# JeffWang987/MVSTER

Measured on AMD Instinct MI355X. Metric: depth-maps/sec (DTU 512×640, 5-view, 4-stage) at 1/2/4/8 MI355X, higher is better.
Workload: dtype f32; 1 GPU; DTU mid 512x640, 5 views, 4-stage cascade 8/8/4/4 hyp, B=1 eval, 1 depth map(s) per step per GPU; launch=hipGraph replay, parallelism=replicas x1, depth_maps_in_flight_per_gpu=2

## Files before the change

mvster_amd/csrc/conv_args.hpp:

```cpp
#pragma once
#include "common.hpp"

namespace mvconv {

typedef float f32x4v __attribute__((ext_vector_type(4)));

constexpr int kMaxTaps = 128;
constexpr int kMaxClasses = 8;

struct ConvArgs {
    const float* in;
    const float* wpk;
    const float* scale;
    const float* shift;
    const float* skip;
    const float* zeros;
    const float* prob_w;
    const float* prob_b;
    float* out;
    int B, Di, Hi, Wi;
    int Do, Ho, Wo;
    int DoF, HoF, WoF;
    int sd, sh, sw;
    int cin;
    int cout;
    int ntile_total;
    int relu;
    int skip_mode;
    int nclass;
    int kd[kMaxClasses], kh[kMaxClasses], kw[kMaxClasses];
    int pd[kMaxClasses], ph[kMaxClasses], pw[kMaxClasses];
    int od[kMaxClasses], oh[kMaxClasses], ow[kMaxClasses];
    int osd, osh, osw;
    int nsteps[kMaxClasses];
    int all_inside[kMaxClasses];
    long woff[kMaxClasses];
    unsigned div_mul[3], div_shr[3];
    unsigned in_bytes;
};

__device__ __forceinline__ unsigned fast_div(unsigned n, unsigned d, unsigned mul, unsigned shr) {
    return d == 1 ? n : (__umulhi(n, mul) >> shr);
}

static inline void find_divisor(unsigned d, unsigned& mul, unsigned& shr) {
    if (d <= 1) { mul = 0; shr = 0; return; }
    int lg = 31 - __builtin_clz(d);
    if (d & (d - 1)) ++lg;
    const int p = 31 + lg;
    mul = (unsigned)(((1ull << p) + d - 1) / d);
    shr = (unsigned)(p - 32);
}

typedef __attribute__((address_space(3))) void lds_void;
typedef unsigned u32x4v __attribute__((ext_vector_type(4)));

struct PersArgs {
    unsigned tiles_x, tiles_y, ntiles;
    unsigned out_bytes;
    int prio;
    unsigned mul[3], shr[3], one[3];
};

struct TilePos { int b, zo, ty0, tx0; };

template <int MT, int KW, int SW, int KD>
struct PersGeom {
    static constexpr int TY = 2 * MT;
    static constexpr int KH = KW;
    static constexpr int PW = 31 * SW + KW;
    static constexpr int PH = (TY - 1) * SW + KH;
    static constexpr int ROWS = KD * PH;
    static constexpr int PWH = (PW + 1) / 2;
    static constexpr int ROWSLOTS = SW == 1 ? PW * 2 : PWH * 4;
    static constexpr int USED = ROWS * ROWSLOTS;
    static constexpr int NBLK = (USED + 63) / 64;
    static constexpr int PLANE = ((NBLK * 64 + 7) & ~7) + 4;
};

static inline bool fill_pers_args(const ConvArgs& a, int TY, PersArgs& p) {
    p.tiles_x = (unsigned)((a.Wo + 31) / 32);
    p.tiles_y = (unsigned)((a.Ho + TY - 1) / TY);
    const long ntiles = (long)p.tiles_x * p.tiles_y * a.Do * a.B;
    const long out_bytes = (long)a.B * a.DoF * a.HoF * a.WoF * a.cout * 4;
    if (ntiles >= (1L << 30) || a.in_bytes >= (1u << 31) || out_bytes >= (1L << 31)) return false;
    p.ntiles = (unsigned)ntiles;
    p.out_bytes = (unsigned)out_bytes;
    p.prio = 0;
    const unsigned divisors[3] = {p.tiles_x, p.tiles_y, (unsigned)a.Do};
    for (int i = 0; i < 3; ++i) {
        find_divisor(divisors[i], p.mul[i], p.shr[i]);
        p.one[i] = divisors[i] == 1 ? ~0u : 0u;
    }
    return true;
}

int num_cus();

static inline bool allow_big_lds(const void* kern, unsigned long& done) {
    int dev = 0;
    if (hipGetDevice(&dev) != hipSuccess) return false;
    if (dev >= 0 && dev < 64 && ((done >> dev) & 1ul)) return true;
    if (hipFuncSetAttribute(kern, hipFuncAttributeMaxDynamicSharedMemorySize, 160 * 1024) != hipSuccess) return false;
    if (dev >= 0 && dev < 64) done |= 1ul << dev;
    return true;
}

int dispatch_pers(const ConvArgs& a, int mt, int nt, int wpc, hipStream_t s);
int dispatch_pp(const ConvArgs& a, int mt, int nt, hipStream_t s);
int dispatch_wino(const ConvArgs& a, int nt, int wpc, bool ring, hipStream_t s);
int dispatch_b3(const ConvArgs& a, int mt, int wpc, hipStream_t s);
int dispatch_1x1(const ConvArgs& a, int mt, int wpc, hipStream_t s);

int dispatch_deconv_select_mfma(const float* in, const float* w, const float* scale, const float* shift, const float* skip,
                                const float* prob_w, const float* prob_b, const float* hypo, float* attn, float* depth,
                                float* conf, float* inv_min, float* inv_max, float* logits_out, int B, int D, int Hi, int Wi,
                                int relu, float split_itv, hipStream_t s);

}
```

mvster_amd/csrc/conv_mfma.hip:

```cpp
#include <stdlib.h>

#include "conv_args.hpp"

namespace {

using namespace mvconv;

typedef unsigned u32x4v __attribute__((ext_vector_type(4)));

#ifdef MVSTER_TIMELINE
__device__ unsigned long long* g_tl = nullptr;
#define MV_TL(k)                                                                                              \
    do {                                                                                                      \
        __builtin_amdgcn_sched_barrier(0);                                                                    \
        if (g_tl && (threadIdx.x & 63) == 0)                                                                  \
            g_tl[((size_t)blockIdx.x * 4 + (threadIdx.x >> 6)) * 8 + (k)] = __builtin_amdgcn_s_memtime();     \
        __builtin_amdgcn_sched_barrier(0);                                                                    \
    } while (0)
#define MV_TL_ID()                                                                                            \
    do {                                                                                                      \
        if (g_tl && (threadIdx.x & 63) == 0) {                                                                \
            g_tl[((size_t)blockIdx.x * 4 + (threadIdx.x >> 6)) * 8 + 6] = __builtin_amdgcn_s_getreg(63492);   \
            g_tl[((size_t)blockIdx.x * 4 + (threadIdx.x >> 6)) * 8 + 7] = __builtin_amdgcn_s_getreg(63508);   \
        }                                                                                                     \
    } while (0)
#else
#define MV_TL(k)
#define MV_TL_ID()
#endif

__device__ __forceinline__ void epilogue_store(const ConvArgs& a, f32x4v v, int n0, long opix, int b, int oy, int ox,
                                               const f32x4v sc, const f32x4v sh) {
    const bool vec = (n0 + 3 < a.cout) && ((a.cout & 3) == 0);
#pragma unroll
    for (int j = 0; j < 4; ++j) {
        v[j] = fmaf(v[j], sc[j], sh[j]);
        if (a.relu) v[j] = fmaxf(v[j], 0.0f);
    }
    if (a.prob_w) {
        if (a.skip_mode == 1) {
            const f32x4v k = *reinterpret_cast<const f32x4v*>(a.skip + opix * a.cout + n0);
#pragma unroll
            for (int j = 0; j < 4; ++j) v[j] += k[j];
        }
        float part = v[0] * a.prob_w[n0];
#pragma unroll
        for (int j = 1; j < 4; ++j) part = fmaf(v[j], a.prob_w[n0 + j], part);
        const float other = __shfl_xor(part, 16);
        if (n0 == 0) a.out[opix] = (part + other) + a.prob_b[0];
        return;
    }
    float* op = a.out + opix * a.cout + n0;
    if (vec) {
        if (a.skip_mode == 1) {
            const f32x4v k = *reinterpret_cast<const f32x4v*>(a.skip + opix * a.cout + n0);
#pragma unroll
            for (int j = 0; j < 4; ++j) v[j] += k[j];
        } else if (a.skip_mode == 2) {
            const int hh = a.HoF / 2, wh = a.WoF / 2;
            const mv::Lerp ly = mv::make_lerp(oy, hh, a.HoF), lx = mv::make_lerp(ox, wh, a.WoF);
            const float* sk = a.skip + (long)b * hh * wh * a.cout + n0;
            const f32x4v k00 = *reinterpret_cast<const f32x4v*>(sk + ((long)ly.i0 * wh + lx.i0) * a.cout);
            const f32x4v k01 = *reinterpret_cast<const f32x4v*>(sk + ((long)ly.i0 * wh + lx.i1) * a.cout);
            const f32x4v k10 = *reinterpret_cast<const f32x4v*>(sk + ((long)ly.i1 * wh + lx.i0) * a.cout);
            const f32x4v k11 = *reinterpret_cast<const f32x4v*>(sk + ((long)ly.i1 * wh + lx.i1) * a.cout);
#pragma unroll
            for (int j = 0; j < 4; ++j) v[j] = mv::bilerp(ly, lx, k00[j], k01[j], k10[j], k11[j]) + v[j];
        }
        *reinterpret_cast<f32x4v*>(op) = v;
    } else {
        for (int j = 0; j < 4; ++j) {
            if (n0 + j >= a.cout) break;
            float r = v[j];
            if (a.skip_mode == 1) r += a.skip[opix * a.cout + n0 + j];
            op[j] = r;
        }
    }
}

__device__ __forceinline__ void epilogue_store(const ConvArgs& a, f32x4v v, int n0, long opix, int b, int oy, int ox) {
    epilogue_store(a, v, n0, opix, b, oy, ox, *reinterpret_cast<const f32x4v*>(a.scale + n0),
                   *reinterpret_cast<const f32x4v*>(a.shift + n0));
}

constexpr int conv_min_waves(int mt, int nt) {
    const int t = mt * nt;
    return t <= 2 ? 5 : (t <= 4 ? 4 : (t <= 8 ? 3 : 2));
}

template <int CIN, int MT, int NT, bool SPLITK>
__global__ void __launch_bounds__(256, conv_min_waves(MT, NT)) conv_mfma_kernel(ConvArgs a) {
    static_assert(CIN % 4 == 0 && (CIN >= 16 ? CIN % 16 == 0 : 16 % CIN == 0), "channel packing");
    __shared__ f32x4v red[SPLITK ? 3 * MT * NT * 64 : 1];
    __shared__ int lut_ofs[kMaxTaps];
    __shared__ int lut_zyx[kMaxTaps];

    const int cls = blockIdx.z;
    const int KD = a.kd[cls], KH = a.kh[cls], KW = a.kw[cls];
    const int ntaps = KD * KH * KW;
    for (int t = threadIdx.x; t < ntaps; t += blockDim.x) {
        const int kx = t % KW, ky = (t / KW) % KH, kz = t / (KW * KH);
        lut_ofs[t] = (kz * a.Hi + ky) * a.Wi + kx;
        lut_zyx[t] = kz | (ky << 8) | (kx << 16);
    }
    __syncthreads();

    const int lane = threadIdx.x & 63;
    const int wave = threadIdx.x >> 6;
    const int lm = lane & 15;
    const int lq = lane >> 4;
    const unsigned Mtot = (unsigned)(a.B * a.Do * a.Ho * a.Wo);
    const int nt0 = blockIdx.y * NT;
    const unsigned ntiles = (Mtot + 15u) >> 4;
    const unsigned ngroups = SPLITK ? (ntiles + MT - 1) / MT : (ntiles + 4 * MT - 1) / (4 * MT);
    for (unsigned grp0 = blockIdx.x; grp0 < ngroups; grp0 += gridDim.x) {
    const unsigned grp = gridDim.x == ngroups ? xcd_remap(grp0, ngroups) : grp0;
    const unsigned tile0 = SPLITK ? grp * MT : (grp * 4u + wave) * MT;
    if (!SPLITK && tile0 * 16u >= Mtot) break;

    int iz0[MT], iy0[MT], ix0[MT];
    int pin0[MT];
    int opix[MT];
    int oyx[MT];
#pragma unroll
    for (int mt = 0; mt < MT; ++mt) {
        unsigned m = (tile0 + mt) * 16u + lm;
        const bool ok = m < Mtot;
        if (!ok) m = 0;
        unsigned r = fast_div(m, a.Wo, a.div_mul[0], a.div_shr[0]);
        const int x = (int)(m - r * (unsigned)a.Wo);
        unsigned r2 = fast_div(r, a.Ho, a.div_mul[1], a.div_shr[1]);
        const int y = (int)(r - r2 * (unsigned)a.Ho);
        const unsigned b = fast_div(r2, a.Do, a.div_mul[2], a.div_shr[2]);
        const int z = (int)(r2 - b * (unsigned)a.Do);
        iz0[mt] = ok ? z * a.sd - a.pd[cls] : -(1 << 20);
        iy0[mt] = y * a.sh - a.ph[cls];
        ix0[mt] = x * a.sw - a.pw[cls];
        pin0[mt] = (((int)b * a.Di + (ok ? iz0[mt] : 0)) * a.Hi + iy0[mt]) * a.Wi + ix0[mt];
        const int oz = z * a.osd + a.od[cls], oy = y * a.osh + a.oh[cls], ox = x * a.osw + a.ow[cls];
        opix[mt] = ok ? (((int)b * a.DoF + oz) * a.HoF + oy) * a.WoF + ox : -1;
        oyx[mt] = (oy << 16) | ox;
    }

    f32x4v acc[MT][NT];
#pragma unroll
    for (int mt = 0; mt < MT; ++mt)
#pragma unroll
        for (int nt = 0; nt < NT; ++nt) acc[mt][nt] = (f32x4v){0.f, 0.f, 0.f, 0.f};

    const float* wp = a.wpk + a.woff[cls] + ((long)nt0 * 64 + lane) * 4;
    const long wstep = (long)a.ntile_total * 256;
    const int nsteps_all = a.nsteps[cls];
    const int kfirst = SPLITK ? wave : 0, kstride = SPLITK ? 4 : 1;
    const int nsteps = SPLITK ? (nsteps_all - wave + 3) / 4 : nsteps_all;

    const __amdgpu_buffer_rsrc_t in_rsrc =
        __builtin_amdgcn_make_buffer_rsrc(const_cast<float*>(a.in), (short)0, (int)a.in_bytes, 0x00020000);
    const bool no_pad = a.all_inside[cls] != 0;
    f32x4v af[MT], bf[NT];
    auto load_step = [&](int si, f32x4v (&A)[MT], f32x4v (&Bv)[NT]) {
        const int s = kfirst + si * kstride;
        const int kk = s * 16 + lq * 4;
        const int tap = kk / CIN;
        const int c = kk % CIN;
        const bool tap_ok = tap < ntaps;
        const int tt = tap_ok ? tap : 0;
        const int ofs = lut_ofs[tt];
        const int zyx = lut_zyx[tt];
        const int kz = zyx & 255, ky = (zyx >> 8) & 255, kx = zyx >> 16;
#pragma unroll
        for (int mt = 0; mt < MT; ++mt) {
            bool ok = tap_ok && iz0[mt] > -(1 << 19);
            if (!no_pad)
                ok = ok && (unsigned)(iz0[mt] + kz) < (unsigned)a.Di && (unsigned)(iy0[mt] + ky) < (unsigned)a.Hi &&
                     (unsigned)(ix0[mt] + kx) < (unsigned)a.Wi;
            const unsigned off = ok ? (unsigned)((pin0[mt] + ofs) * CIN + c) * 4u : 0xFFFFFFF0u;
            A[mt] = __builtin_bit_cast(f32x4v, __builtin_amdgcn_raw_buffer_load_b128(in_rsrc, off, 0, 0));
        }
#pragma unroll
        for (int nt = 0; nt < NT; ++nt)
            Bv[nt] = *reinterpret_cast<const f32x4v*>(wp + (long)s * wstep + (long)nt * 256);
    };

    auto mma_step = [&](const f32x4v (&A)[MT], const f32x4v (&Bv)[NT]) {
#pragma unroll
        for (int j = 0; j < 4; ++j)
#pragma unroll
            for (int mt = 0; mt < MT; ++mt)
#pragma unroll
                for (int nt = 0; nt < NT; ++nt)
                    acc[mt][nt] = __builtin_amdgcn_mfma_f32_16x16x4f32(Bv[nt][j], A[mt][j], acc[mt][nt], 0, 0, 0);
    };

    f32x4v ag[MT], bg[NT];
    if (nsteps > 0) {
        load_step(0, af, bf);
        int s = 0;
        for (; s + 2 <= nsteps; s += 2) {
            load_step(s + 1, ag, bg);
            mma_step(af, bf);
            load_step(s + 2 < nsteps ? s + 2 : nsteps - 1, af, bf);
            mma_step(ag, bg);
        }
        if (s < nsteps) mma_step(af, bf);
    }

    if (SPLITK) {
        if (wave > 0) {
#pragma unroll
            for (int mt = 0; mt < MT; ++mt)
#pragma unroll
                for (int nt = 0; nt < NT; ++nt) red[((wave - 1) * MT * NT + mt * NT + nt) * 64 + lane] = acc[mt][nt];
        }
        __syncthreads();
        if (wave > 0) return;
#pragma unroll
        for (int w = 0; w < 3; ++w)
#pragma unroll
            for (int mt = 0; mt < MT; ++mt)
#pragma unroll
                for (int nt = 0; nt < NT; ++nt) {
                    const f32x4v r = red[(w * MT * NT + mt * NT + nt) * 64 + lane];
#pragma unroll
                    for (int j = 0; j < 4; ++j) acc[mt][nt][j] += r[j];
                }
    }

#pragma unroll
    for (int mt = 0; mt < MT; ++mt) {
        if (opix[mt] < 0) continue;
        const int b = a.skip_mode == 2 ? opix[mt] / (a.DoF * a.HoF * a.WoF) : 0;
#pragma unroll
        for (int nt = 0; nt < NT; ++nt) {
            const int n0 = (nt0 + nt) * 16 + lq * 4;
            if (n0 >= a.cout) continue;
            epilogue_store(a, acc[mt][nt], n0, opix[mt], b, oyx[mt] >> 16, oyx[mt] & 0xffff);
        }
    }
    }
}

template <int CIN, int MT, int NT, bool SPLITK>
int launch(const ConvArgs& a, hipStream_t s) {
    const long Mtot = (long)a.B * a.Do * a.Ho * a.Wo;
    if (Mtot >= (1L << 31) || (long)a.B * a.Di * a.Hi * a.Wi >= (1L << 31)) return MVSTER_ERR_SHAPE;
    const long tiles = (Mtot + 15) / 16;
    const long per_block = SPLITK ? MT : 4 * MT;
    long gx = (tiles + per_block - 1) / per_block;
    dim3 grid((unsigned)gx, a.ntile_total / NT, a.nclass);
    MV_NOTE_KERNEL("conv_mfma_kernel<%d, %d, %d, %s>", CIN, MT, NT, SPLITK ? "true" : "false");
    hipLaunchKernelGGL((conv_mfma_kernel<CIN, MT, NT, SPLITK>), grid, dim3(256), 0, s, a);
    return mv_check_launch();
}

template <int CIN>
int dispatch_tiles(const ConvArgs& a, int MT, int NT, bool splitk, hipStream_t s) {
    if (splitk) {
        if constexpr (CIN >= 16) {
#define MV_S(M_, N_) if (MT == M_ && NT == N_) return launch<CIN, M_, N_, true>(a, s);
            MV_S(1, 1) MV_S(1, 2) MV_S(1, 4) MV_S(2, 1) MV_S(2, 2)
#undef MV_S
        }
        return MVSTER_ERR_UNSUPPORTED;
    }
#define MV_T(M_, N_) if (MT == M_ && NT == N_) return launch<CIN, M_, N_, false>(a, s);
    MV_T(1, 1) MV_T(2, 1) MV_T(4, 1) MV_T(1, 2) MV_T(2, 2) MV_T(4, 2) MV_T(1, 4) MV_T(2, 4) MV_T(4, 4)
    if constexpr (CIN == 64) {
        MV_T(1, 5) MV_T(2, 5) MV_T(4, 5)
        MV_T(1, 3) MV_T(2, 3) MV_T(4, 3) MV_T(1, 9) MV_T(2, 9)
    }
#undef MV_T
    return MVSTER_ERR_UNSUPPORTED;
}

struct LdsDivs {
    unsigned mul[6], shr[6];
};
constexpr int kMaxStage = 12;
__device__ __forceinline__ int patch_plane(int npix) { return ((npix * 2 + 7) & ~7) + 4; }
static const bool g_no_wlds = MV_PROBE_ENV("MVSTER_NO_WLDS") != nullptr;

template <int MT, int NT, int KW, int NG, int WN>
__global__ void __launch_bounds__(256) conv_lds_kernel(ConvArgs a, int tiles_x, int tiles_y, LdsDivs dv) {
    extern __shared__ __attribute__((aligned(16))) float patch_raw[];
    MV_TL(0);
    MV_TL_ID();
    f32x4v* patch_base = reinterpret_cast<f32x4v*>(patch_raw);
    f32x4v* wl = patch_base + NG * 1024 + 32;
    constexpr int TY = 2 * MT;
    const int KD = a.kd[0], KH = a.kh[0];
    const int PW = 31 * a.sw + KW, PH = (TY - 1) * a.sh + KH;
    const int CIN = a.cin, nchunks = CIN >> 4;
    const int plane = patch_plane(KD * PH * PW);

    unsigned bid = xcd_remap(blockIdx.x, gridDim.x);
    unsigned q = fast_div(bid, tiles_x, dv.mul[0], dv.shr[0]);
    const int tile_x = bid - q * tiles_x; bid = q;
    q = fast_div(bid, tiles_y, dv.mul[1], dv.shr[1]);
    const int tile_y = bid - q * tiles_y; bid = q;
    q = fast_div(bid, a.Do, dv.mul[2], dv.shr[2]);
    const int zo = bid - q * a.Do;
    const int b = q;
    const int ty0 = tile_y * TY, tx0 = tile_x * 32;
    const int nt0 = blockIdx.y * NT;

    const int lane = threadIdx.x & 63, wave = threadIdx.x >> 6;
    const int lm = lane & 15, lq = lane >> 4;

    const bool split = a.sw == 2;
    const int PWH = (PW + 1) >> 1;
    const int npix = KD * PH * PW;
    int goff[NG], gslot[NG];
#pragma unroll
    for (int g = 0; g < NG; ++g) {
        const unsigned pix = threadIdx.x + g * 256;
        int off = -1;
        gslot[g] = (int)pix;
        if ((int)pix < npix) {
            const unsigned prow = fast_div(pix, PW, dv.mul[3], dv.shr[3]);
            const int px = pix - prow * PW;
            if (split) gslot[g] = (int)(prow * PW) + (px & 1) * PWH + (px >> 1);
            const int pz = fast_div(prow, PH, dv.mul[4], dv.shr[4]);
            const int py = prow - pz * PH;
            const int iz = zo * a.sd - a.pd[0] + pz, iy = ty0 * a.sh - a.ph[0] + py, ix = tx0 * a.sw - a.pw[0] + px;
            if ((unsigned)iz < (unsigned)a.Di && (unsigned)iy < (unsigned)a.Hi && (unsigned)ix < (unsigned)a.Wi)
                off = (((b * a.Di + iz) * a.Hi + iy) * a.Wi + ix) * CIN;
        }
        goff[g] = off;
    }
    const long zero_off = a.zeros - a.in;

    const float* wp = a.wpk + ((long)nt0 * 64 + lane) * 4;
    const long wstep = (long)a.ntile_total * 256;

    f32x4v stg[NG * 4];
    constexpr bool WL = WN > 0;
    f32x4v wst[WL ? WN : 1];
    const int nW = KD * KH * KW * NT * 64;
    auto stage_load = [&](int ch) {
#pragma unroll
        for (int i = 0; i < NG * 4; ++i) {
            const int o = goff[i >> 2];
            const long off = o >= 0 ? (long)o + ch * 16 + (i & 3) * 4 : zero_off;
            stg[i] = *reinterpret_cast<const f32x4v*>(a.in + off);
        }
        if (WL) {
#pragma unroll
            for (int i = 0; i < WN; ++i) {
                const int idx = min((int)threadIdx.x + i * 256, nW - 1);
                const int t = idx / (NT * 64), rem = idx - t * (NT * 64);
                wst[i] = *reinterpret_cast<const f32x4v*>(a.wpk + (long)(t * nchunks + ch) * wstep + ((long)nt0 * 64 + rem) * 4);
            }
        }
    };
    auto stage_store = [&](f32x4v* dst) {
#pragma unroll
        for (int i = 0; i < NG * 4; ++i) {
            const int pix = threadIdx.x + (i >> 2) * 256, quad = i & 3;
            if (pix < npix) dst[(quad >> 1) * plane + gslot[i >> 2] * 2 + (quad & 1)] = stg[i];
        }
        if (WL) {
#pragma unroll
            for (int i = 0; i < WN; ++i) wl[threadIdx.x + i * 256] = wst[i];
        }
    };
    stage_load(0);
    int abase[MT];
#pragma unroll
    for (int mt = 0; mt < MT; ++mt) {
        const int t = wave * MT + mt;
        const int row = t >> 1, xs = t & 1;
        abase[mt] = ((row * a.sh) * PW + (xs * 16 + lm) * (split ? 1 : a.sw)) * 2 + (lq >> 1) * plane + (lq & 1);
    }
    int kxo[KW];
#pragma unroll
    for (int kx = 0; kx < KW; ++kx) kxo[kx] = split ? ((kx & 1) * PWH + (kx >> 1)) * 2 : kx * 2;

    f32x4v acc[MT][NT];
#pragma unroll
    for (int mt = 0; mt < MT; ++mt)
#pragma unroll
        for (int nt = 0; nt < NT; ++nt) acc[mt][nt] = (f32x4v){0.f, 0.f, 0.f, 0.f};

    f32x4v scv[NT], shv[NT];
#pragma unroll
    for (int nt = 0; nt < NT; ++nt) {
        const int n0 = min((nt0 + nt) * 16 + lq * 4, a.ntile_total * 16 - 4);
        scv[nt] = *reinterpret_cast<const f32x4v*>(a.scale + n0);
        shv[nt] = *reinterpret_cast<const f32x4v*>(a.shift + n0);
    }
    MV_TL(1);
    stage_store(patch_base);
    MV_TL(2);
    __syncthreads();
    MV_TL(3);
    for (int ch = 0; ch < nchunks; ++ch) {
        const f32x4v* patch = patch_base;
        if (ch + 1 < nchunks) stage_load(ch + 1);
        const int kz_lo = max(0, a.pd[0] - zo * a.sd), kz_hi = min(KD, a.Di + a.pd[0] - zo * a.sd);
        const int r_first = kz_lo * KH, nrows = kz_hi * KH;
        auto load_row = [&](int r, f32x4v (&A)[KW][MT], f32x4v (&Bv)[KW][NT]) {
            const int kz = fast_div(r, KH, dv.mul[5], dv.shr[5]), ky = r - kz * KH;
            const int rowoff = (kz * PH + ky) * PW * 2;
            const float* w = wp + (long)(r * KW * nchunks + ch) * wstep;
#pragma unroll
            for (int kx = 0; kx < KW; ++kx) {
#pragma unroll
                for (int mt = 0; mt < MT; ++mt) A[kx][mt] = patch[abase[mt] + rowoff + kxo[kx]];
#pragma unroll
                for (int nt = 0; nt < NT; ++nt)
                    Bv[kx][nt] = WL ? wl[((r * KW + kx) * NT + nt) * 64 + lane]
                                    : *reinterpret_cast<const f32x4v*>(w + (long)kx * nchunks * wstep + nt * 256);
            }
        };
        auto mma_row = [&](const f32x4v (&A)[KW][MT], const f32x4v (&Bv)[KW][NT]) {
#pragma unroll
            for (int kx = 0; kx < KW; ++kx)
#pragma unroll
                for (int j = 0; j < 4; ++j)
#pragma unroll
                    for (int mt = 0; mt < MT; ++mt)
#pragma unroll
                        for (int nt = 0; nt < NT; ++nt)
                            acc[mt][nt] = __builtin_amdgcn_mfma_f32_16x16x4f32(Bv[kx][nt][j], A[kx][mt][j], acc[mt][nt], 0, 0, 0);
        };
        f32x4v a0[KW][MT], b0[KW][NT], a1[KW][MT], b1[KW][NT];
        load_row(r_first, a0, b0);
        int r = r_first;
        for (; r + 2 <= nrows; r += 2) {
            load_row(r + 1, a1, b1);
            mma_row(a0, b0);
            load_row(r + 2 < nrows ? r + 2 : nrows - 1, a0, b0);
            mma_row(a1, b1);
        }
        if (r < nrows) mma_row(a0, b0);
        if (ch + 1 < nchunks) {
            __syncthreads();
            stage_store(patch_base);
            __syncthreads();
        }
    }

    MV_TL(4);
#pragma unroll
    for (int mt = 0; mt < MT; ++mt) {
        const int t = wave * MT + mt;
        const int y = ty0 + (t >> 1), x = tx0 + (t & 1) * 16 + lm;
        if (y >= a.Ho || x >= a.Wo) continue;
        const long opix = (((long)b * a.Do + zo) * a.Ho + y) * a.Wo + x;
#pragma unroll
        for (int nt = 0; nt < NT; ++nt) {
            const int n0 = (nt0 + nt) * 16 + lq * 4;
            if (n0 >= a.cout) continue;
            epilogue_store(a, acc[mt][nt], n0, opix, b, y, x, scv[nt], shv[nt]);
        }
    }
    MV_TL(5);
}

template <int MT, int NT, int KW, int NG>
int launch_lds_ng(const ConvArgs& a, int tiles_x, int tiles_y, hipStream_t s) {
    const long blocks = (long)tiles_x * tiles_y * a.Do * a.B;
    if (blocks >= (1L << 31) || (long)a.B * a.Di * a.Hi * a.Wi * a.cin >= (1L << 31)) return MVSTER_ERR_SHAPE;
    dim3 grid((unsigned)blocks, a.ntile_total / NT, 1);
    LdsDivs dv;
    const unsigned divisors[6] = {(unsigned)tiles_x, (unsigned)tiles_y, (unsigned)a.Do, (unsigned)(31 * a.sw + KW),
                                  (unsigned)((2 * MT - 1) * a.sh + a.kh[0]), (unsigned)a.kh[0]};
    for (int i = 0; i < 6; ++i) find_divisor(divisors[i], dv.mul[i], dv.shr[i]);
    const int nw = a.kd[0] * a.kh[0] * KW * NT * 64;
    if (nw <= 3 * 256 && !g_no_wlds) {
        const size_t lds = (size_t)(NG * 1024 + 32) * 16 + 3 * 256 * 16;
        MV_NOTE_KERNEL("conv_lds_kernel<%d, %d, %d, %d, 3>", MT, NT, KW, NG);
        hipLaunchKernelGGL((conv_lds_kernel<MT, NT, KW, NG, 3>), grid, dim3(256), lds, s, a, tiles_x, tiles_y, dv);
    } else {
        const size_t lds = (size_t)(NG * 1024 + 32) * 16;
        MV_NOTE_KERNEL("conv_lds_kernel<%d, %d, %d, %d, 0>", MT, NT, KW, NG);
        hipLaunchKernelGGL((conv_lds_kernel<MT, NT, KW, NG, 0>), grid, dim3(256), lds, s, a, tiles_x, tiles_y, dv);
    }
    return mv_check_launch();
}

template <int MT, int NT, int KW>
int launch_lds(const ConvArgs& a, hipStream_t s) {
    constexpr int TY = 2 * MT;
    const int PW = 31 * a.sw + KW, PH = (TY - 1) * a.sh + a.kh[0];
    const size_t nstage = (size_t)a.kd[0] * PH * PW * 4;
    if (nstage > (size_t)kMaxStage * 256) return MVSTER_ERR_SHAPE;
    const int tiles_x = (a.Wo + 31) / 32, tiles_y = (a.Ho + TY - 1) / TY;
    const int ng = (int)((nstage + 1023) / 1024);
    if (ng == 1) return launch_lds_ng<MT, NT, KW, 1>(a, tiles_x, tiles_y, s);
    if (ng == 2) return launch_lds_ng<MT, NT, KW, 2>(a, tiles_x, tiles_y, s);
    return launch_lds_ng<MT, NT, KW, 3>(a, tiles_x, tiles_y, s);
}

int dispatch_lds(const ConvArgs& a, int MT, int NT, hipStream_t s) {
    if (a.nclass != 1 || a.cin % 16 != 0 || a.skip_mode > 1 || a.osd != 1 || a.osh != 1 || a.osw != 1)
        return MVSTER_ERR_UNSUPPORTED;
#define MV_L(M_, N_, K_) if (MT == M_ && NT == N_ && a.kw[0] == K_) return launch_lds<M_, N_, K_>(a, s);
    MV_L(2, 1, 3) MV_L(2, 2, 3) MV_L(2, 4, 3) MV_L(4, 1, 3) MV_L(4, 2, 3) MV_L(4, 4, 3)
    MV_L(2, 1, 5) MV_L(2, 2, 5) MV_L(2, 4, 5) MV_L(4, 1, 5) MV_L(4, 2, 5) MV_L(4, 4, 5)
#undef MV_L
    return MVSTER_ERR_UNSUPPORTED;
}

__global__ void mfma_probe_kernel(const float* A, const float* Bm, float* Dm) {
    const int lane = threadIdx.x;
    f32x4v acc = {0.f, 0.f, 0.f, 0.f};
    const float av = A[(lane & 15) * 4 + (lane >> 4)];
    const float bv = Bm[(lane >> 4) * 16 + (lane & 15)];
    acc = __builtin_amdgcn_mfma_f32_16x16x4f32(av, bv, acc, 0, 0, 0);
    for (int r = 0; r < 4; ++r) Dm[((lane >> 4) * 4 + r) * 16 + (lane & 15)] = acc[r];
}

}

extern "C" int mvster_conv_mfma(const float* in, const float* wpk, const float* scale, const float* shift,
                                const float* skip, const float* zeros, const float* prob_w, const float* prob_b,
                                float* out, const int* geom, int ngeom, const long* woff, int cin, int mt, int nt,
                                int variant, void* stream) {
    if (!in || !wpk || !scale || !shift || !zeros || !out || !geom || !woff) return MVSTER_ERR_NULL;
    if (ngeom < 22) return MVSTER_ERR_SHAPE;
    ConvArgs a;
    a.in = in; a.wpk = wpk; a.scale = scale; a.shift = shift; a.skip = skip; a.zeros = zeros; a.out = out;
    a.prob_w = prob_w; a.prob_b = prob_b;
    if ((prob_w == nullptr) != (prob_b == nullptr)) return MVSTER_ERR_NULL;
    int i = 0;
    a.B = geom[i++]; a.Di = geom[i++]; a.Hi = geom[i++]; a.Wi = geom[i++];
    a.Do = geom[i++]; a.Ho = geom[i++]; a.Wo = geom[i++];
    a.DoF = geom[i++]; a.HoF = geom[i++]; a.WoF = geom[i++];
    a.sd = geom[i++]; a.sh = geom[i++]; a.sw = geom[i++];
    a.cout = geom[i++]; a.ntile_total = geom[i++]; a.relu = geom[i++]; a.skip_mode = geom[i++];
    a.osd = geom[i++]; a.osh = geom[i++]; a.osw = geom[i++];
    a.nclass = geom[i++];
    if (a.nclass < 1 || a.nclass > kMaxClasses || ngeom < i + a.nclass * 10) return MVSTER_ERR_SHAPE;
    for (int c = 0; c < a.nclass; ++c) {
        a.kd[c] = geom[i++]; a.kh[c] = geom[i++]; a.kw[c] = geom[i++];
        a.pd[c] = geom[i++]; a.ph[c] = geom[i++]; a.pw[c] = geom[i++];
        a.od[c] = geom[i++]; a.oh[c] = geom[i++]; a.ow[c] = geom[i++];
        a.nsteps[c] = geom[i++];
        a.woff[c] = woff[c];
        if (a.kd[c] * a.kh[c] * a.kw[c] > kMaxTaps || a.nsteps[c] < 1) return MVSTER_ERR_SHAPE;
    }
    if (a.B <= 0 || a.Do <= 0 || a.Ho <= 0 || a.Wo <= 0 || a.cout <= 0 || a.ntile_total <= 0) return MVSTER_ERR_SHAPE;
    find_divisor((unsigned)a.Wo, a.div_mul[0], a.div_shr[0]);
    find_divisor((unsigned)a.Ho, a.div_mul[1], a.div_shr[1]);
    find_divisor((unsigned)a.Do, a.div_mul[2], a.div_shr[2]);
    {
        const long in_elems = (long)a.B * a.Di * a.Hi * a.Wi * cin;
        const long out_elems = (long)a.B * a.DoF * a.HoF * a.WoF * a.cout;
        if (in_elems >= (1L << 30) || out_elems >= (1L << 31)) return MVSTER_ERR_SHAPE;
        a.in_bytes = (unsigned)(in_elems * 4);
    }
    for (int c = 0; c < a.nclass; ++c) {
        auto inside = [](int n_out, int s, int p, int k, int extent) {
            return -p >= 0 && (n_out - 1) * s - p + (k - 1) < extent;
        };
        a.all_inside[c] = inside(a.Do, a.sd, a.pd[c], a.kd[c], a.Di) && inside(a.Ho, a.sh, a.ph[c], a.kh[c], a.Hi) &&
                          inside(a.Wo, a.sw, a.pw[c], a.kw[c], a.Wi);
    }
    if (a.skip_mode != 0 && !skip) return MVSTER_ERR_NULL;
    if (a.ntile_total % nt != 0) return MVSTER_ERR_SHAPE;
    hipStream_t s = (hipStream_t)stream;
    a.cin = cin;
    if ((variant & 0xff) == 5) return dispatch_pers(a, mt, nt, variant >> 8, s);
    if ((variant & 0xff) == 6) return dispatch_1x1(a, mt, variant >> 8, s);
    if ((variant & 0xff) == 7) return dispatch_pp(a, mt, nt, s);
    if ((variant & 0xff) == 8) return dispatch_wino(a, nt, variant >> 8, false, s);
    if ((variant & 0xff) == 9) return dispatch_wino(a, nt, variant >> 8, true, s);
    if ((variant & 0xff) == 11) return dispatch_b3(a, mt, variant >> 8, s);
    if (prob_w && (a.cout != 8 || a.skip_mode == 2 || variant == 1)) return MVSTER_ERR_UNSUPPORTED;
    if (variant == 1) return dispatch_lds(a, mt, nt, s);
    if (variant != 0 && variant != 2) return MVSTER_ERR_UNSUPPORTED;
    const bool splitk = variant == 2;
    switch (cin) {
        case 4: return dispatch_tiles<4>(a, mt, nt, splitk, s);
        case 8: return dispatch_tiles<8>(a, mt, nt, splitk, s);
        case 16: return dispatch_tiles<16>(a, mt, nt, splitk, s);
        case 32: return dispatch_tiles<32>(a, mt, nt, splitk, s);
        case 64: return dispatch_tiles<64>(a, mt, nt, splitk, s);
        case 80: return dispatch_tiles<80>(a, mt, nt, splitk, s);
        default: return MVSTER_ERR_UNSUPPORTED;
    }
}

#ifdef MVSTER_TIMELINE
extern "C" int mvster_debug_timeline(void* buf) {
    return hipMemcpyToSymbol(HIP_SYMBOL(g_tl), &buf, sizeof(buf)) == hipSuccess ? MVSTER_OK : MVSTER_ERR_LAUNCH;
}
#endif

extern "C" int mvster_mfma_probe(const float* A, const float* B, float* D, void* stream) {
    if (!A || !B || !D) return MVSTER_ERR_NULL;
    hipLaunchKernelGGL(mfma_probe_kernel, dim3(1), dim3(64), 0, (hipStream_t)stream, A, B, D);
    return mv_check_launch();
}

namespace {
__global__ void __launch_bounds__(256) pack_weights_kernel(const float* __restrict__ w, float* __restrict__ wpk, int nsteps,
                                                           int ntile, int cout, int cin, int cin_pad, int kd, int kh, int kw,
                                                           long s_n, long s_c, long s_z, long s_y, long s_x, int flip) {
    const int idx = blockIdx.x * 256 + threadIdx.x;
    if (idx >= nsteps * ntile * 64) return;
    const int lane = idx & 63, t = (idx >> 6) % ntile, st = (idx >> 6) / ntile;
    const int n = t * 16 + (lane & 15);
    const int ntaps = kd * kh * kw;
    f32x4v out;
#pragma unroll
    for (int j = 0; j < 4; ++j) {
        const int k = st * 16 + (lane >> 4) * 4 + j;
        const int tap = k / cin_pad, ci = k - tap * cin_pad;
        float v = 0.0f;
        if (tap < ntaps && ci < cin && n < cout) {
            int kx = tap % kw, ky = (tap / kw) % kh, kz = tap / (kw * kh);
            if (flip) { kx = kw - 1 - kx; ky = kh - 1 - ky; kz = kd - 1 - kz; }
            v = w[(long)n * s_n + (long)ci * s_c + (long)kz * s_z + (long)ky * s_y + (long)kx * s_x];
        }
        out[j] = v;
    }
    *reinterpret_cast<f32x4v*>(wpk + (long)idx * 4) = out;
}
}

namespace {
struct PackClasses {
    int nclass;
    int ntaps[kMaxClasses];
    long woff[kMaxClasses];
    unsigned char tap[kMaxClasses][27];
};

__global__ void __launch_bounds__(256) pack_weights_classes_kernel(const float* __restrict__ w, float* __restrict__ wpk,
                                                                   PackClasses pc, int ntile, int cout, int cin, int cin_pad,
                                                                   int ktot) {
    const int cls = blockIdx.y;
    const int ntaps = pc.ntaps[cls];
    const int nsteps = (ntaps * cin_pad + 15) / 16;
    const int idx = blockIdx.x * 256 + threadIdx.x;
    if (idx >= nsteps * ntile * 64) return;
    const int lane = idx & 63, t = (idx >> 6) % ntile, st = (idx >> 6) / ntile;
    const int n = t * 16 + (lane & 15);
    f32x4v out;
#pragma unroll
    for (int j = 0; j < 4; ++j) {
        const int k = st * 16 + (lane >> 4) * 4 + j;
        const int tl = k / cin_pad, ci = k - tl * cin_pad;
        float v = 0.0f;
        if (tl < ntaps && ci < cin && n < cout) v = w[((long)ci * cout + n) * ktot + pc.tap[cls][tl]];
        out[j] = v;
    }
    *reinterpret_cast<f32x4v*>(wpk + pc.woff[cls] + (long)idx * 4) = out;
}
}

extern "C" int mvster_pack_conv_weights_classes(const float* w, float* wpk, int cout, int cin, int cin_pad, int ktot, int nclass,
                                                const int* ntaps, const long* woff, const int* taps, void* stream) {
    if (!w || !wpk || !ntaps || !woff || !taps) return MVSTER_ERR_NULL;
    if (cout <= 0 || cin <= 0 || cin_pad < cin || ktot <= 0 || ktot > 27 || nclass <= 0 || nclass > kMaxClasses)
        return MVSTER_ERR_SHAPE;
    PackClasses pc;
    pc.nclass = nclass;
    int maxsteps = 0;
    for (int c = 0; c < nclass; ++c) {
        if (ntaps[c] <= 0 || ntaps[c] > 27) return MVSTER_ERR_SHAPE;
        pc.ntaps[c] = ntaps[c];
        pc.woff[c] = woff[c];
        for (int t = 0; t < 27; ++t) pc.tap[c][t] = (unsigned char)(t < ntaps[c] ? taps[c * 27 + t] : 0);
        const int ns = (ntaps[c] * cin_pad + 15) / 16;
        maxsteps = ns > maxsteps ? ns : maxsteps;
    }
    const int ntile = (cout + 15) / 16;
    const int total = maxsteps * ntile * 64;
    hipLaunchKernelGGL(pack_weights_classes_kernel, dim3((total + 255) / 256, nclass), dim3(256), 0, (hipStream_t)stream, w, wpk,
                       pc, ntile, cout, cin, cin_pad, ktot);
    return mv_check_launch();
}

extern "C" int mvster_pack_conv_weights(const float* w, float* wpk, int cout, int cin, int cin_pad, int kd, int kh, int kw,
                                        long s_n, long s_c, long s_z, long s_y, long s_x, int flip, void* stream) {
    if (!w || !wpk) return MVSTER_ERR_NULL;
    if (cout <= 0 || cin <= 0 || cin_pad < cin || kd <= 0 || kh <= 0 || kw <= 0) return MVSTER_ERR_SHAPE;
    const int nsteps = (kd * kh * kw * cin_pad + 15) / 16, ntile = (cout + 15) / 16;
    const int total = nsteps * ntile * 64;
    hipLaunchKernelGGL(pack_weights_kernel, dim3((total + 255) / 256), dim3(256), 0, (hipStream_t)stream, w, wpk, nsteps, ntile,
                       cout, cin, cin_pad, kd, kh, kw, s_n, s_c, s_z, s_y, s_x, flip);
    return mv_check_launch();
}
```

Measured before the change: 1149 depth-maps/s.

## Replace LDS tap LUT with magic-division decode and per-voxel bounds bitmasks

Removes the shared-memory tap lookup table and its block-wide barrier from the generic MFMA conv kernel. Taps are now decoded with precomputed magic-number division, and padding checks use a per-output-voxel axis bitmask tested against a per-tap select mask. When there is no padding and CIN≥16 the loop uses wave-uniform scalar offsets in the buffer load. Weight loads also move to buffer loads with a scalar offset. This cuts LDS traffic, the barrier and per-step VALU address math, at the cost of more template specialisation and a separate unpipelined fallback for large kernels.

```diff
diff --git a/mvster_amd/csrc/conv_args.hpp b/mvster_amd/csrc/conv_args.hpp
--- a/mvster_amd/csrc/conv_args.hpp
+++ b/mvster_amd/csrc/conv_args.hpp
@@ -1,5 +1,6 @@
 #pragma once
 #include "common.hpp"
+#include "conv_taps.h"
 
 namespace mvconv {
 
@@ -37,6 +38,7 @@
     long woff[kMaxClasses];
     unsigned div_mul[3], div_shr[3];
     unsigned in_bytes;
+    mvtaps::TapDivs tapdiv[kMaxClasses];
 };
 
 __device__ __forceinline__ unsigned fast_div(unsigned n, unsigned d, unsigned mul, unsigned shr) {
diff --git a/mvster_amd/csrc/conv_mfma.hip b/mvster_amd/csrc/conv_mfma.hip
--- a/mvster_amd/csrc/conv_mfma.hip
+++ b/mvster_amd/csrc/conv_mfma.hip
@@ -1,4 +1,6 @@
 #include <stdlib.h>
+
+#include <type_traits>
 
 #include "conv_args.hpp"
 
@@ -92,21 +94,18 @@
 __global__ void __launch_bounds__(256, conv_min_waves(MT, NT)) conv_mfma_kernel(ConvArgs a) {
     static_assert(CIN % 4 == 0 && (CIN >= 16 ? CIN % 16 == 0 : 16 % CIN == 0), "channel packing");
     __shared__ f32x4v red[SPLITK ? 3 * MT * NT * 64 : 1];
-    __shared__ int lut_ofs[kMaxTaps];
-    __shared__ int lut_zyx[kMaxTaps];
 
     const int cls = blockIdx.z;
     const int KD = a.kd[cls], KH = a.kh[cls], KW = a.kw[cls];
+    const int PD = a.pd[cls], PH = a.ph[cls], PW = a.pw[cls];
     const int ntaps = KD * KH * KW;
-    for (int t = threadIdx.x; t < ntaps; t += blockDim.x) {
-        const int kx = t % KW, ky = (t / KW) % KH, kz = t / (KW * KH);
-        lut_ofs[t] = (kz * a.Hi + ky) * a.Wi + kx;
-        lut_zyx[t] = kz | (ky << 8) | (kx << 16);
-    }
-    __syncthreads();
+    const mvtaps::TapDivs tdv = a.tapdiv[cls];
+    const int nsteps_all = a.nsteps[cls];
+    const bool no_pad = a.all_inside[cls] != 0;
+    const bool fit = mvtaps::masks_fit(KD, KH, KW);
 
     const int lane = threadIdx.x & 63;
-    const int wave = threadIdx.x >> 6;
+    const int wave = __builtin_amdgcn_readfirstlane(threadIdx.x >> 6);
     const int lm = lane & 15;
     const int lq = lane >> 4;
     const unsigned Mtot = (unsigned)(a.B * a.Do * a.Ho * a.Wo);
@@ -119,7 +118,8 @@
     if (!SPLITK && tile0 * 16u >= Mtot) break;
 
     int iz0[MT], iy0[MT], ix0[MT];
-    int pin0[MT];
+    unsigned abase[MT];
+    unsigned vmask[MT];
     int opix[MT];
     int oyx[MT];
 #pragma unroll
@@ -133,10 +133,12 @@
         const int y = (int)(r - r2 * (unsigned)a.Ho);
         const unsigned b = fast_div(r2, a.Do, a.div_mul[2], a.div_shr[2]);
         const int z = (int)(r2 - b * (unsigned)a.Do);
-        iz0[mt] = ok ? z * a.sd - a.pd[cls] : -(1 << 20);
-        iy0[mt] = y * a.sh - a.ph[cls];
-        ix0[mt] = x * a.sw - a.pw[cls];
-        pin0[mt] = (((int)b * a.Di + (ok ? iz0[mt] : 0)) * a.Hi + iy0[mt]) * a.Wi + ix0[mt];
+        iz0[mt] = ok ? z * a.sd - PD : -(1 << 20);
+        iy0[mt] = y * a.sh - PH;
+        ix0[mt] = x * a.sw - PW;
+        const int pin0 = (((int)b * a.Di + (ok ? iz0[mt] : 0)) * a.Hi + iy0[mt]) * a.Wi + ix0[mt];
+        abase[mt] = (unsigned)(pin0 * CIN + (CIN >= 16 ? lq * 4 : 0)) * 4u;
+        vmask[mt] = fit ? mvtaps::voxel_mask(iz0[mt], iy0[mt], ix0[mt], KD, KH, KW, a.Di, a.Hi, a.Wi) : 0u;
         const int oz = z * a.osd + a.od[cls], oy = y * a.osh + a.oh[cls], ox = x * a.osw + a.ow[cls];
         opix[mt] = ok ? (((int)b * a.DoF + oz) * a.HoF + oy) * a.WoF + ox : -1;
         oyx[mt] = (oy << 16) | ox;
@@ -148,38 +150,41 @@
 #pragma unroll
         for (int nt = 0; nt < NT; ++nt) acc[mt][nt] = (f32x4v){0.f, 0.f, 0.f, 0.f};
 
-    const float* wp = a.wpk + a.woff[cls] + ((long)nt0 * 64 + lane) * 4;
-    const long wstep = (long)a.ntile_total * 256;
-    const int nsteps_all = a.nsteps[cls];
-    const int kfirst = SPLITK ? wave : 0, kstride = SPLITK ? 4 : 1;
-    const int nsteps = SPLITK ? (nsteps_all - wave + 3) / 4 : nsteps_all;
+    const long wstep = (long)a.ntile_total * 1024;
+    const __amdgpu_buffer_rsrc_t w_rsrc = __builtin_amdgcn_make_buffer_rsrc(
+        const_cast<float*>(a.wpk + a.woff[cls] + (long)nt0 * 256), (short)0,
+        (int)((unsigned)nsteps_all * (unsigned)wstep - (unsigned)nt0 * 1024u), 0x00020000);
+    const unsigned wlane = (unsigned)lane * 16u;
 
     const __amdgpu_buffer_rsrc_t in_rsrc =
         __builtin_amdgcn_make_buffer_rsrc(const_cast<float*>(a.in), (short)0, (int)a.in_bytes, 0x00020000);
-    const bool no_pad = a.all_inside[cls] != 0;
-    f32x4v af[MT], bf[NT];
-    auto load_step = [&](int si, f32x4v (&A)[MT], f32x4v (&Bv)[NT]) {
-        const int s = kfirst + si * kstride;
-        const int kk = s * 16 + lq * 4;
-        const int tap = kk / CIN;
-        const int c = kk % CIN;
-        const bool tap_ok = tap < ntaps;
-        const int tt = tap_ok ? tap : 0;
-        const int ofs = lut_ofs[tt];
-        const int zyx = lut_zyx[tt];
-        const int kz = zyx & 255, ky = (zyx >> 8) & 255, kx = zyx >> 16;
+    const int nsteps = mvtaps::wave_steps(nsteps_all, wave, SPLITK);
+
+    auto uni = [](unsigned v) { return CIN >= 16 ? (unsigned)__builtin_amdgcn_readfirstlane((int)v) : v; };
+    auto load_step = [&](auto mode, int si, f32x4v (&A)[MT], f32x4v (&Bv)[NT]) {
+        constexpr int MODE = decltype(mode)::value;
+        const int s = mvtaps::wave_step(si, wave, SPLITK);
+        const int tap = mvtaps::step_tap<CIN>(s, lq);
+        const int c = CIN >= 16 ? s * 16 - tap * CIN : mvtaps::step_channel<CIN>(s, lq);
+        const bool tap_ok = CIN >= 16 || tap < ntaps;
+        const mvtaps::Tap t = mvtaps::tap_decode(tap_ok ? tap : 0, KH, KW, tdv);
+        const unsigned uoff = uni((unsigned)(mvtaps::tap_offset(t, a.Hi, a.Wi) * CIN + c) * 4u);
+        const unsigned sel = MODE == 1 ? uni(mvtaps::tap_select(t, KD, KH)) : 0u;
 #pragma unroll
         for (int mt = 0; mt < MT; ++mt) {
-            bool ok = tap_ok && iz0[mt] > -(1 << 19);
-            if (!no_pad)
-                ok = ok && (unsigned)(iz0[mt] + kz) < (unsigned)a.Di && (unsigned)(iy0[mt] + ky) < (unsigned)a.Hi &&
-                     (unsigned)(ix0[mt] + kx) < (unsigned)a.Wi;
-            const unsigned off = ok ? (unsigned)((pin0[mt] + ofs) * CIN + c) * 4u : 0xFFFFFFF0u;
-            A[mt] = __builtin_bit_cast(f32x4v, __builtin_amdgcn_raw_buffer_load_b128(in_rsrc, off, 0, 0));
-        }
+            if constexpr (MODE == 0) {
+                A[mt] = __builtin_bit_cast(f32x4v, __builtin_amdgcn_raw_buffer_load_b128(in_rsrc, abase[mt], uoff, 0));
+            } else {
+                const bool ok = tap_ok && (MODE == 1 ? mvtaps::tap_inside(vmask[mt], sel)
+                                                     : mvtaps::tap_inside_cmp(iz0[mt], iy0[mt], ix0[mt], t, a.Di, a.Hi, a.Wi));
+                const unsigned off = ok ? abase[mt] + uoff : 0xFFFFFFF0u;
+                A[mt] = __builtin_bit_cast(f32x4v, __builtin_amdgcn_raw_buffer_load_b128(in_rsrc, off, 0, 0));
+            }
+        }
+        const unsigned woff = (unsigned)s * (unsigned)wstep;
 #pragma unroll
         for (int nt = 0; nt < NT; ++nt)
-            Bv[nt] = *reinterpret_cast<const f32x4v*>(wp + (long)s * wstep + (long)nt * 256);
+            Bv[nt] = __builtin_bit_cast(f32x4v, __builtin_amdgcn_raw_buffer_load_b128(w_rsrc, wlane + nt * 1024u, woff, 0));
     };
 
     auto mma_step = [&](const f32x4v (&A)[MT], const f32x4v (&Bv)[NT]) {
@@ -192,17 +197,30 @@
                     acc[mt][nt] = __builtin_amdgcn_mfma_f32_16x16x4f32(Bv[nt][j], A[mt][j], acc[mt][nt], 0, 0, 0);
     };
 
-    f32x4v ag[MT], bg[NT];
-    if (nsteps > 0) {
-        load_step(0, af, bf);
+    auto k_loop = [&](auto mode) {
+        f32x4v af[MT], bf[NT], ag[MT], bg[NT];
+        if (nsteps <= 0) return;
+        const int last = nsteps - 1;
+        load_step(mode, 0, af, bf);
         int s = 0;
         for (; s + 2 <= nsteps; s += 2) {
-            load_step(s + 1, ag, bg);
+            load_step(mode, s + 1, ag, bg);
             mma_step(af, bf);
-            load_step(s + 2 < nsteps ? s + 2 : nsteps - 1, af, bf);
+            load_step(mode, min(s + 2, last), af, bf);
             mma_step(ag, bg);
         }
         if (s < nsteps) mma_step(af, bf);
+    };
+    if (!fit) {
+        f32x4v af[MT], bf[NT];
+        for (int s = 0; s < nsteps; ++s) {
+            load_step(std::integral_constant<int, 2>{}, s, af, bf);
+            mma_step(af, bf);
+        }
+    } else if (CIN >= 16 && no_pad) {
+        k_loop(std::integral_constant<int, CIN >= 16 ? 0 : 1>{});
+    } else {
+        k_loop(std::integral_constant<int, 1>{});
     }
 
     if (SPLITK) {
@@ -540,6 +558,8 @@
         a.nsteps[c] = geom[i++];
         a.woff[c] = woff[c];
         if (a.kd[c] * a.kh[c] * a.kw[c] > kMaxTaps || a.nsteps[c] < 1) return MVSTER_ERR_SHAPE;
+        if (a.kd[c] < 1 || a.kh[c] < 1 || a.kw[c] < 1) return MVSTER_ERR_SHAPE;
+        a.tapdiv[c] = mvtaps::make_tap_divs(a.kh[c], a.kw[c]);
     }
     if (a.B <= 0 || a.Do <= 0 || a.Ho <= 0 || a.Wo <= 0 || a.cout <= 0 || a.ntile_total <= 0) return MVSTER_ERR_SHAPE;
     find_divisor((unsigned)a.Wo, a.div_mul[0], a.div_shr[0]);
diff --git a/mvster_amd/csrc/conv_taps.h b/mvster_amd/csrc/conv_taps.h
--- /dev/null
+++ b/mvster_amd/csrc/conv_taps.h
@@ -0,0 +1,88 @@
+#pragma once
+
+#if defined(__HIPCC__)
+#define MVT_HD __host__ __device__ __forceinline__
+#else
+#define MVT_HD inline
+#endif
+
+namespace mvtaps {
+
+struct TapDivs {
+    unsigned kw_mul, kw_shr, kw_one, kh_mul, kh_shr, kh_one;
+};
+
+struct Tap {
+    int kz, ky, kx;
+};
+
+MVT_HD unsigned mulhi(unsigned a, unsigned b) { return (unsigned)(((unsigned long long)a * b) >> 32); }
+
+MVT_HD unsigned div_ms(unsigned n, unsigned mul, unsigned shr, unsigned one) { return (mulhi(n, mul) >> shr) | (n & one); }
+
+inline void make_tap_div(int d, unsigned& mul, unsigned& shr, unsigned& one) {
+    mul = 0u; shr = 0u; one = ~0u;
+    if (d <= 1) return;
+    int lg = 31 - __builtin_clz((unsigned)d);
+    if (d & (d - 1)) ++lg;
+    const int p = 31 + lg;
+    mul = (unsigned)(((1ull << p) + (unsigned)d - 1) / (unsigned)d);
+    shr = (unsigned)(p - 32);
+    one = 0u;
+}
+inline TapDivs make_tap_divs(int KH, int KW) {
+    TapDivs dv;
+    make_tap_div(KW, dv.kw_mul, dv.kw_shr, dv.kw_one);
+    make_tap_div(KH, dv.kh_mul, dv.kh_shr, dv.kh_one);
+    return dv;
+}
+
+template <int CIN>
+MVT_HD int step_tap(int s, int lq) {
+    return (int)(CIN >= 16 ? ((unsigned)s * 16u) / (unsigned)CIN : ((unsigned)s * 16u + (unsigned)lq * 4u) / (unsigned)CIN);
+}
+template <int CIN>
+MVT_HD int step_channel(int s, int lq) {
+    return (int)(((unsigned)s * 16u + (unsigned)lq * 4u) % (unsigned)CIN);
+}
+
+MVT_HD Tap tap_decode(int tap, int KH, int KW, const TapDivs& dv) {
+    const unsigned r = div_ms((unsigned)tap, dv.kw_mul, dv.kw_shr, dv.kw_one);
+    const unsigned z = div_ms(r, dv.kh_mul, dv.kh_shr, dv.kh_one);
+    Tap t;
+    t.kx = tap - (int)r * KW;
+    t.ky = (int)r - (int)z * KH;
+    t.kz = (int)z;
+    return t;
+}
+
+MVT_HD int tap_offset(const Tap& t, int Hi, int Wi) { return (t.kz * Hi + t.ky) * Wi + t.kx; }
+
+MVT_HD bool masks_fit(int KD, int KH, int KW) { return KD + KH + KW <= 32; }
+
+MVT_HD unsigned axis_mask(int i0, int K, int extent) {
+    const int lo = i0 < 0 ? -i0 : 0;
+    const int hi = extent - i0 < K ? extent - i0 : K;
+    if (hi <= lo) return 0u;
+    return ((1u << hi) - 1u) & ~((1u << lo) - 1u);
+}
+
+MVT_HD unsigned voxel_mask(int iz0, int iy0, int ix0, int KD, int KH, int KW, int Di, int Hi, int Wi) {
+    return axis_mask(iz0, KD, Di) | (axis_mask(iy0, KH, Hi) << KD) | (axis_mask(ix0, KW, Wi) << (KD + KH));
+}
+
+MVT_HD unsigned tap_select(const Tap& t, int KD, int KH) {
+    return (1u << t.kz) | (1u << (KD + t.ky)) | (1u << (KD + KH + t.kx));
+}
+
+MVT_HD bool tap_inside(unsigned vmask, unsigned sel) { return (vmask & sel) == sel; }
+
+MVT_HD bool tap_inside_cmp(int iz0, int iy0, int ix0, const Tap& t, int Di, int Hi, int Wi) {
+    return (unsigned)(iz0 + t.kz) < (unsigned)Di && (unsigned)(iy0 + t.ky) < (unsigned)Hi &&
+           (unsigned)(ix0 + t.kx) < (unsigned)Wi;
+}
+
+MVT_HD int wave_steps(int nsteps_all, int wave, bool splitk) { return splitk ? (nsteps_all - wave + 3) / 4 : nsteps_all; }
+MVT_HD int wave_step(int si, int wave, bool splitk) { return splitk ? wave + 4 * si : si; }
+
+}
```

After: 1167 depth-maps/s, median of 6. 1.5% higher.
